# ImIntheMiddle/VATL4Pose-WACV2024

Measured on AMD Instinct MI355X. Metric: frames/sec pose-infer+uncertainty, 256x192 17-kp, higher is better.
Workload: dtype f32; 1 GPU; SimpleBaseline-R50 256x192 inference + decode + local-peak + THC-L1, 1024-frame synthetic video per GPU; frames_per_gpu=1024, batch=1024, tracks=4, parallelism=frame-sharded x1

## Files before the change

### include/vatl_hip.h

```cpp
#ifndef VATL_HIP_H
#define VATL_HIP_H

#include <stdint.h>

#ifdef __cplusplus
extern "C" {
#endif

#define VATL_VERSION 100
#define VATL_EINVAL  (-1)
#define VATL_ELAUNCH (-2)

int         vatl_version(void);
const char* vatl_last_error(void);

int vatl_flop_meter_begin(void);
int vatl_flop_meter_end(double* direct_flops, double* winograd_flops, int64_t* direct_launches, int64_t* winograd_launches);
#define VATL_ROUTE_NAMES "igemm,igemm_bnbwd,igemm_dma,persistent_1x1,streamk,rows_1x1,bottleneck_chain,stem_pool,halo_3x3," \
                         "winograd,winograd_2h,winograd_bnbwd,winograd_persist,winograd_c32,wgrad,winograd_wgrad,winograd_wgrad_2h," \
                         "winograd_wgrad_table,winograd_f4,winograd_f4_bnbwd,gemm1x1_ring"
int vatl_flop_meter_routes(int64_t* counts, int n);


int vatl_nchw_to_nhwc(const float* src, float* dst, int N, int C, int H, int W, int Cpad, void* stream);
int vatl_nhwc_to_nchw(const float* src, float* dst, int N, int C, int H, int W, void* stream);

int vatl_pack_conv_weight(const float* w_oihw, float* w_packed, int Cout, int Cin, int R, int S,
                          int CoutPad, int Spad, int CinPad, void* stream);
int vatl_pack_deconv4x4s2_weight(const float* w_iohw, float* w_packed, int Cin, int Cout, int CoutPad, void* stream);
int64_t vatl_stem_pool_weight_floats(void);
int vatl_pack_stem_pool_weight(const float* w_oihw, float* packed, void* stream);
int vatl_stem_pool_supported(int H, int W);
int vatl_stem7x7s2_pool_fwd(const float* x_nchw, const float* w_packed, const float* scale, const float* bias, float* y_nhwc,
                            int N, int H, int W, void* stream);
int64_t vatl_stem3_weight_floats(void);
int vatl_pack_stem3_weight(const float* w_oihw, float* packed, void* stream);
int vatl_stem3x3s2_fwd(const float* x_nchw, const float* w_packed, const float* scale, const float* bias, float* y_nhwc,
                       int N, int H, int W, void* stream);

int vatl_bn_fold(const float* gamma, const float* beta, const float* mean, const float* var, const float* conv_bias,
                 float eps, float* scale, float* bias, int C, void* stream);


int vatl_pack_conv1x1_dual_weight(const float* w1, const float* scale1, const float* bias1, const float* w2, const float* scale2,
                                  const float* bias2, float* out, float* bias, int Cout, int C1, int C2, int CoutPad, void* stream);
int vatl_conv1x1_dual_fwd(const float* a, const float* x, const float* w, const float* bias, float* y, int N, int Ho, int Wo,
                          int C1, int H2, int W2, int C2, int stride2, int Cout, int CoutPad, int relu, void* stream);

int64_t vatl_winograd_c32_weight_floats(void);
int vatl_pack_winograd_c32_weight(const float* w, float* u, void* stream);
int vatl_conv3x3_winograd_c32_supported(int N, int H, int W, int Cin, int Cout);
int vatl_conv3x3_winograd_c32_fwd(const float* x, const float* u, const float* scale, const float* bias, const float* residual, float* y, int N, int H, int W,
                                  int relu, void* stream);

int64_t vatl_winograd_f4_weight_floats(int Cout, int Cin);
int vatl_pack_winograd_f4_weight(const float* w, float* u, int Cout, int Cin, int data_gradient, void* stream);
int vatl_conv3x3_winograd_f4_supported(int N, int H, int W, int Cin, int Cout);
int vatl_conv3x3_winograd_f4_fwd(const float* x, const float* u, const float* scale, const float* bias, const float* residual, float* y, int N, int H, int W,
                                 int Cin, int Cout, int relu, void* stream);
int64_t vatl_winograd_f4_stats_row_blocks(int64_t N, int H, int W);
int vatl_conv3x3_winograd_f4_fwd_stats(const float* x, const float* u, float* y, double* stats, int64_t* row_blocks_used, int N, int H, int W, int Cin, int Cout,
                                       void* stream);
int vatl_conv3x3_winograd_f4_fwd_bnbwd(const float* x, const float* u, const float* residual, float* y, int N, int H, int W, int Cin, int Cout, const float* bn_z,
                                       const float* bn_mask_y, const float* bn_scale, const float* bn_bias, const float* bn_mean, const float* bn_invstd,
                                       double* stats, int64_t* row_blocks_used, void* stream);

int vatl_conv1x1_rows_supported(int K1, int K2, int N, int64_t M);
int vatl_conv1x1_rows_fwd(const float* a, const float* x2, const float* w, const float* scale, const float* bias, const float* residual, float* y,
                          int64_t M, int K1, int K2, int N, int relu, void* stream);

int vatl_bottleneck_chain_supported(int Cmid, int Cout, int Cnext, int64_t M);
int vatl_bottleneck_chain_fwd(const float* a, const float* w3, const float* scale3, const float* bias3, const float* skip, float* t,
                              const float* w1, const float* scale1, const float* bias1, float* y1, int64_t M, int Cmid, int Cout,
// ... 200 lines not shown
```

### vatl4pose-wacv2024_amd/csrc/common.h

```cpp
#pragma once
#include <hip/hip_runtime.h>
#include <atomic>
#include <cstdarg>
#include <cstdio>
#include <cstdint>

#include "vatl_hip.h"

namespace vatl {

char* err_buf();
int fail(int code, const char* fmt, ...);

void meter_add(int kind, double flops);
enum MeterRoute {
    kRouteIgemm = 0, kRouteIgemmBnBwd, kRouteIgemmDma, kRoutePersistent1x1, kRouteStreamK, kRouteRows, kRouteChain, kRouteStemPool, kRouteHalo,
    kRouteWino, kRouteWino2H, kRouteWinoBnBwd, kRouteWinoPersist, kRouteWinoC32, kRouteWgrad, kRouteWinoWgrad, kRouteWinoWgrad2H,
    kRouteWinoWgradTable, kRouteWinoF4, kRouteWinoF4BnBwd, kRouteGemm1x1Ring, kRouteCount
};
void meter_route(int route);

inline int check_launch(const char* what) {
    hipError_t e = hipGetLastError();
    if (e != hipSuccess) return fail(VATL_ELAUNCH, "%s: %s", what, hipGetErrorString(e));
    return 0;
}

inline int ensure_dynamic_lds(const void* kern, int bytes, std::atomic<unsigned>& done_mask, const char* what) {
    int d = 0;
    if (hipGetDevice(&d) != hipSuccess) return fail(VATL_ELAUNCH, "%s: no current device", what);
    const unsigned bit = 1u << (d & 31);
    if (done_mask.load(std::memory_order_acquire) & bit) return 0;
    hipError_t e = hipFuncSetAttribute(kern, hipFuncAttributeMaxDynamicSharedMemorySize, bytes);
    if (e != hipSuccess) return fail(VATL_ELAUNCH, "hipFuncSetAttribute(%s): %s", what, hipGetErrorString(e));
    done_mask.fetch_or(bit, std::memory_order_release);
    return 0;
}

static inline int cdiv(int64_t a, int64_t b) { return (int)((a + b - 1) / b); }

typedef float f32x4 __attribute__((ext_vector_type(4)));
typedef float f32x16 __attribute__((ext_vector_type(16)));

__device__ __forceinline__ void lds_barrier() {
    asm volatile("s_waitcnt lgkmcnt(0)" ::: "memory");
    __builtin_amdgcn_s_barrier();
    asm volatile("" ::: "memory");
}

__device__ __forceinline__ float wave_sum(float v) {
#pragma unroll
    for (int o = 32; o > 0; o >>= 1) v += __shfl_xor(v, o, 64);
    return v;
}
__device__ __forceinline__ double wave_sum(double v) {
#pragma unroll
    for (int o = 32; o > 0; o >>= 1) v += __shfl_xor(v, o, 64);
    return v;
}
__device__ __forceinline__ float wave_max(float v) {
#pragma unroll
    for (int o = 32; o > 0; o >>= 1) v = fmaxf(v, __shfl_xor(v, o, 64));
    return v;
}
__device__ __forceinline__ int wave_sum(int v) {
#pragma unroll
    for (int o = 32; o > 0; o >>= 1) v += __shfl_xor(v, o, 64);
    return v;
}

__device__ __forceinline__ int fast_div(int q, float inv_w) { return (int)(((float)q + 0.5f) * inv_w); }
// ... 16 lines not shown
```

### vatl4pose-wacv2024_amd/csrc/conv_igemm.hip

```cpp
#include "common.h"

#include <algorithm>
#include <atomic>
#include <cstdlib>

namespace vatl {

struct ConvParams {
    const float* x;
    const float* w;
    const float* scale;
    const float* bias;
    const float* res;
    float* y;
    int N, H, W, Cin;
    int Cout, CoutPad;
    int R, S, stride, pad_y, pad_x;
    int Ho, Wo, M;
    int OH, OW, osy, osx, ooy, oox;
    int relu, out_nchw, deconv;
    int kpr;
    int ktiles;
    int n_tiles, m_tiles;
    int order;
// ... 1052 lines not shown

    constexpr int NG = BK / 8;
    constexpr int MPG = 4 * TM * TN;
    for (int kt = 0; kt < p.ktiles; ++kt) {
        const int buf = kt & 1;
        f32x4 af[2][TM], bf[2][TN];
        frag_read(af[0], bf[0], buf, 0);
#pragma unroll
        for (int g = 0; g < NG; ++g) {
            if (g + 1 < NG) frag_read(af[(g + 1) & 1], bf[(g + 1) & 1], buf, g + 1);
            if (g == 0) issue(buf ^ 1, kt + 1);
#pragma unroll
            for (int tt = 0; tt < 4; ++tt)
#pragma unroll
                for (int i = 0; i < TM; ++i)
#pragma unroll
                    for (int j = 0; j < TN; ++j)
                        acc[i][j] = __builtin_amdgcn_mfma_f32_32x32x2f32(af[g & 1][i][tt], bf[g & 1][j][tt], acc[i][j], 0, 0, 0);
            if (g + 1 < NG) __builtin_amdgcn_sched_group_barrier(0x100, TM + TN, 0);
#pragma unroll
            for (int q2 = 0; q2 < MPG; ++q2) {
                __builtin_amdgcn_sched_group_barrier(0x008, 1, 0);
                __builtin_amdgcn_sched_group_barrier(0x016, 2, 0);
            }
            __builtin_amdgcn_sched_barrier(0);
        }
        asm volatile("s_waitcnt vmcnt(0)" ::: "memory");
        __syncthreads();
    }
    conv_epilogue<BM, BN, WM, WN>(p, acc, smem, m0, n0, ooy, oox, wm, wn, tid, lane, HoWo);
}

template <int BM, int BN, int WM, int WN>
__global__ __launch_bounds__(256, 2) void conv_igemm_dma_kernel(ConvParams p) {
    extern __shared__ __attribute__((aligned(16))) float smem[];
    conv_igemm_dma_body<BM, BN, WM, WN>(p, smem);
}

constexpr int RING_BK = 16;
constexpr int RING_NS = 4;
constexpr int RING_STAGE = 256 * RING_BK;
constexpr int RING_BYTES = RING_NS * RING_STAGE * (int)sizeof(float);

template <int N>
__device__ __forceinline__ void ring_wait_vm() {
    static_assert(N == 0 || N == 4 || N == 8 || N == 32 || N == 36, "add the count here");
    if constexpr (N == 0) asm volatile("s_waitcnt vmcnt(0)" ::: "memory");
    else if constexpr (N == 4) asm volatile("s_waitcnt vmcnt(4)" ::: "memory");
    else if constexpr (N == 8) asm volatile("s_waitcnt vmcnt(8)" ::: "memory");
    else if constexpr (N == 32) asm volatile("s_waitcnt vmcnt(32)" ::: "memory");
    else asm volatile("s_waitcnt vmcnt(36)" ::: "memory");
}

template <bool DUAL, bool RES>
__device__ __forceinline__ void gemm1x1_ring_body(const ConvParams& p, float* smem) {
    const int tid = threadIdx.x, lane = tid & 63;
    const int wave = __builtin_amdgcn_readfirstlane(tid >> 6);
    const int wm = wave >> 1, wn = wave & 1;

    const int nblk = gridDim.x, bid = blockIdx.x;
    const int xcd = bid & 7, loc = bid >> 3, q = nblk >> 3, r8 = nblk & 7;
    const int t = (xcd < r8 ? xcd * (q + 1) : r8 * (q + 1) + (xcd - r8) * q) + loc;
    const int m_tile = t / p.n_tiles, n_tile = t - m_tile * p.n_tiles;
    const int m0 = m_tile * 128, n0 = n_tile * 128;

    const __amdgpu_buffer_rsrc_t xr = __builtin_amdgcn_make_buffer_rsrc(const_cast<float*>(p.x), 0, p.x_bytes, 0x00020000);
    const __amdgpu_buffer_rsrc_t wr = __builtin_amdgcn_make_buffer_rsrc(const_cast<float*>(p.w), 0, p.w_bytes, 0x00020000);
    const __amdgpu_buffer_rsrc_t xr2 = __builtin_amdgcn_make_buffer_rsrc(const_cast<float*>(DUAL ? p.x2 : p.x), 0, DUAL ? p.x2_bytes : p.x_bytes, 0x00020000);

    const int lchk = (lane & 3) ^ ((lane >> 4) & 3);
    unsigned aoff[2], boff[2], aoff2[2];
#pragma unroll
    for (int u = 0; u < 2; ++u) {
        const int row = (4 * u + wave) * 16 + (lane >> 2);
        const int m = min(m0 + row, p.M - 1);
        aoff[u] = (unsigned)m * (unsigned)(p.Cin * 4) + (unsigned)lchk * 16u;
        aoff2[u] = 0;
        if (DUAL) {
            const int b = fdiv(m, p.d_HoWo);
            const int rem = m - b * p.Ho * p.Wo;
            const int oy = fdiv(rem, p.d_Wo);
            const int ox = rem - oy * p.Wo;
            aoff2[u] = (unsigned)((b * p.H2 + oy * p.stride2) * p.W2 + ox * p.stride2) * (unsigned)(p.C2 * 4) + (unsigned)lchk * 16u;
        }
        boff[u] = (unsigned)(n0 + row) * (unsigned)(p.K * 4) + (unsigned)lchk * 16u;
    }
    const int S = p.ktiles * 2;
    const int S1 = DUAL ? p.k1 * 2 : S;
    auto issue = [&](auto src, int buf, int s) {
        float* st = smem + buf * RING_STAGE;
#pragma unroll
        for (int u = 0; u < 2; ++u) {
            lds_void* da = (lds_void*)(st + (4 * u + wave) * 256);
            if constexpr (DUAL && decltype(src)::value == 1) __builtin_amdgcn_raw_ptr_buffer_load_lds(xr2, da, 16, aoff2[u], (unsigned)(s - S1) * 64u, 0, 0);
            else                                             __builtin_amdgcn_raw_ptr_buffer_load_lds(xr, da, 16, aoff[u], (unsigned)s * 64u, 0, 0);
        }
#pragma unroll
        for (int u = 0; u < 2; ++u)
            __builtin_amdgcn_raw_ptr_buffer_load_lds(wr, (lds_void*)(st + 128 * RING_BK + (4 * u + wave) * 256), 16, boff[u], (unsigned)s * 64u, 0, 0);
    };

    const int frow = lane & 31, h = lane >> 5;
    const int fsw = (frow >> 2) & 3;
    const float* Ard[2];
    const float* Brd[2];
#pragma unroll
    for (int g = 0; g < 2; ++g) {
        Ard[g] = smem + (wm * 64 + frow) * RING_BK + (((2 * g + h) ^ fsw) << 2);
        Brd[g] = smem + 128 * RING_BK + (wn * 64 + frow) * RING_BK + (((2 * g + h) ^ fsw) << 2);
    }

    const unsigned rowb = (unsigned)p.Cout * 4u;
    const unsigned ylane = (unsigned)(m0 + wm * 64 + 4 * h) * rowb + (unsigned)(n0 + wn * 64 + frow) * 4u;
    float sc[2], bi[2];
#pragma unroll
    for (int j = 0; j < 2; ++j) {
        const int n = n0 + wn * 64 + j * 32 + frow;
        sc[j] = p.scale ? p.scale[n] : 1.f;
        bi[j] = p.bias ? p.bias[n] : 0.f;
    }
    const __amdgpu_buffer_rsrc_t yr = __builtin_amdgcn_make_buffer_rsrc(p.y, 0, p.y_bytes, 0x00020000);
    const __amdgpu_buffer_rsrc_t rr = __builtin_amdgcn_make_buffer_rsrc(const_cast<float*>(RES ? p.res : p.y), 0, RES ? p.y_bytes : 0u, 0x00020000);
    float rs[2][2][16];
#pragma unroll
    for (int i = 0; i < 2; ++i)
#pragma unroll
        for (int j = 0; j < 2; ++j)
#pragma unroll
            for (int e = 0; e < 16; ++e) rs[i][j][e] = 0.f;
    auto res_load = [&](int i) {
#pragma unroll
        for (int j = 0; j < 2; ++j)
#pragma unroll
            for (int e = 0; e < 16; ++e)
                rs[i][j][e] = __builtin_bit_cast(float, __builtin_amdgcn_raw_buffer_load_b32(
                                  rr, ylane + (unsigned)(32 * i + (e & 3) + 8 * (e >> 2)) * rowb + (unsigned)j * 128u, 0, 0));
    };

    f32x16 acc[2][2];
#pragma unroll
    for (int i = 0; i < 2; ++i)
#pragma unroll
        for (int j = 0; j < 2; ++j)
#pragma unroll
            for (int e = 0; e < 16; ++e) acc[i][j][e] = 0.f;

    auto stage = [&](auto slot, auto kind, auto src, int s) {
        constexpr int B = decltype(slot)::value, KIND = decltype(kind)::value;
        if constexpr (KIND <= 1) ring_wait_vm<8>();
        else if constexpr (KIND == 2) ring_wait_vm<RES ? 36 : 4>();
        else ring_wait_vm<RES ? 32 : 0>();
        __builtin_amdgcn_s_barrier();
        asm volatile("" ::: "memory");
        f32x4 af[2][2], bf[2][2];
#pragma unroll
        for (int g = 0; g < 2; ++g)
#pragma unroll
            for (int i = 0; i < 2; ++i) {
                af[g][i] = *reinterpret_cast<const f32x4*>(Ard[g] + B * RING_STAGE + i * 32 * RING_BK);
                bf[g][i] = *reinterpret_cast<const f32x4*>(Brd[g] + B * RING_STAGE + i * 32 * RING_BK);
            }
        if constexpr (KIND == 0) issue(src, (B + 3) & 3, s + 3);
        if constexpr (RES && KIND == 1) res_load(0);
        if constexpr (RES && KIND == 3) res_load(1);
#pragma unroll
        for (int g = 0; g < 2; ++g)
#pragma unroll
            for (int tt = 0; tt < 4; ++tt)
#pragma unroll
                for (int i = 0; i < 2; ++i)
#pragma unroll
                    for (int j = 0; j < 2; ++j)
                        acc[i][j] = __builtin_amdgcn_mfma_f32_32x32x2f32(af[g][i][tt], bf[g][j][tt], acc[i][j], 0, 0, 0);
        __builtin_amdgcn_sched_group_barrier(0x100, 8, 0);
        if constexpr (KIND == 0) {
#pragma unroll
            for (int k = 0; k < 4; ++k) {
                __builtin_amdgcn_sched_group_barrier(0x008, 1, 0);
                __builtin_amdgcn_sched_group_barrier(0x020, 1, 0);
            }
            __builtin_amdgcn_sched_group_barrier(0x008, 28, 0);
        }
        __builtin_amdgcn_sched_barrier(0);
    };
    using C0 = std::integral_constant<int, 0>;
    using C1 = std::integral_constant<int, 1>;
    using C2 = std::integral_constant<int, 2>;
    using C3 = std::integral_constant<int, 3>;

    using X2 = std::integral_constant<int, DUAL ? 1 : 0>;
    auto group = [&](auto src, int s) {
        stage(C0{}, C0{}, src, s);
        stage(C1{}, C0{}, src, s + 1);
        stage(C2{}, C0{}, src, s + 2);
        stage(C3{}, C0{}, src, s + 3);
    };

    issue(C0{}, 0, 0);
    issue(C0{}, 1, 1);
    issue(C0{}, 2, 2);
    int s = 0;
    if constexpr (DUAL) {
        for (; s < S1 - 4; s += 4) group(C0{}, s);
        stage(C0{}, C0{}, C0{}, s);
        stage(C1{}, C0{}, X2{}, s + 1);
        stage(C2{}, C0{}, X2{}, s + 2);
        stage(C3{}, C0{}, X2{}, s + 3);
        s += 4;
    }
    for (; s < S - 4; s += 4) group(X2{}, s);
    stage(C0{}, C0{}, X2{}, s);
    stage(C1{}, C1{}, X2{}, s + 1);
    stage(C2{}, C2{}, X2{}, s + 2);
    stage(C3{}, C3{}, X2{}, s + 3);

    const float lo = p.relu ? 0.f : -INFINITY;
#pragma unroll
    for (int i = 0; i < 2; ++i)
#pragma unroll
        for (int j = 0; j < 2; ++j)
#pragma unroll
            for (int e = 0; e < 16; ++e) {
                const float v = fmaxf(acc[i][j][e] * sc[j] + bi[j] + rs[i][j][e], lo);
                __builtin_amdgcn_raw_buffer_store_b32(__builtin_bit_cast(unsigned, v), yr,
                                                      ylane + (unsigned)(32 * i + (e & 3) + 8 * (e >> 2)) * rowb + (unsigned)j * 128u, 0, 0);
            }
}

template <bool DUAL, bool RES>
__global__ __launch_bounds__(256, 2) void gemm1x1_ring_kernel(ConvParams p) {
    extern __shared__ __attribute__((aligned(16))) float smem[];
    gemm1x1_ring_body<DUAL, RES>(p, smem);
}

template <int BM, int BN, int WM, int WN>
static int launch_dma(const ConvParams& p, int phases, hipStream_t st);

static std::atomic<int> g_var{4};
static std::atomic<int> g_order{0};
static std::atomic<int> g_ablate{0};
static std::atomic<int> g_bm{0};
static std::atomic<int> g_stagger{0};
static std::atomic<int> g_splitk_policy{0};

__global__ void splitk_reduce_kernel(const float* __restrict__ part, long long slice, int splits, const float* __restrict__ scale,
                                     const float* __restrict__ bias, const float* __restrict__ res, float* __restrict__ y, long long total, int Cout,
                                     int OHW, int relu, int out_nchw) {
    for (long long i = blockIdx.x * (long long)blockDim.x + threadIdx.x; i < total; i += (long long)gridDim.x * blockDim.x) {
        const int c = (int)(i % Cout);
        float v = 0.f;
        for (int z = 0; z < splits; ++z) v += part[(long long)z * slice + i];
        v = v * (scale ? scale[c] : 1.f) + (bias ? bias[c] : 0.f);
        long long o = i;
        if (out_nchw) {
            const long long pix = i / Cout;
            const long long b = pix / OHW;
            o = (b * Cout + c) * OHW + (pix - b * OHW);
        }
        if (res) v += res[o];
        y[o] = relu ? fmaxf(v, 0.f) : v;
    }
}

constexpr int kMaxDevices = 16;
static std::atomic<float*> g_splitk_ws[kMaxDevices];
static std::atomic<long long> g_splitk_floats[kMaxDevices];
static std::atomic<int> g_splitk_any{0};

static thread_local float* tl_splitk_ws = nullptr;
static thread_local long long tl_splitk_floats = 0;

static float* splitk_workspace(long long* floats, int* policy) {
    if (tl_splitk_ws) { *floats = tl_splitk_floats; *policy = 1; return tl_splitk_ws; }
    *policy = g_splitk_policy.load(std::memory_order_relaxed);
    if (!g_splitk_any.load(std::memory_order_acquire)) return nullptr;
    int d = 0;
    if (hipGetDevice(&d) != hipSuccess || d < 0 || d >= kMaxDevices) return nullptr;
    *floats = g_splitk_floats[d].load(std::memory_order_relaxed);
    return g_splitk_ws[d].load(std::memory_order_acquire);
}

template <int BM, int BN, int WM, int WN, bool STEM, int VAR, bool DUAL = false, int NT = 256, bool BNB = false>
static int launch(const ConvParams& p, int phases, hipStream_t st) {
    auto kern = conv_igemm_kernel<BM, BN, WM, WN, STEM, VAR, DUAL, NT, BNB>;
    constexpr int smem = conv_smem_floats(BM, BN) * (int)sizeof(float);
// ... 58 lines not shown
    auto kern = conv_igemm_dma_kernel<BM, BN, WM, WN>;
    constexpr int stage_bytes = 2 * (BM + BN) * BK * (int)sizeof(float);
    constexpr int epi_bytes = BM * (BN + 4) * (int)sizeof(float);
    constexpr int smem = stage_bytes > epi_bytes ? stage_bytes : epi_bytes;
    static std::atomic<unsigned> configured{0};
    if (int rc = ensure_dynamic_lds(reinterpret_cast<const void*>(kern), smem, configured, "conv_igemm_dma")) return rc;
    ConvParams q = p;
    q.n_tiles = p.CoutPad / BN;
    q.m_tiles = cdiv(p.M, BM);
    q.order = 0; q.stagger = 0;
    dim3 grid((unsigned)(q.m_tiles * q.n_tiles), (unsigned)phases, 1);
    hipLaunchKernelGGL(kern, grid, dim3(256), smem, st, q);
    meter_add(0, 2.0 * ((double)q.m_tiles * BM) * ((double)q.n_tiles * BN) * ((double)q.ktiles * BK) * phases);
    meter_route(kRouteIgemmDma);
    return check_launch("conv_igemm_dma");
}

static std::atomic<int> g_persist_dist{2};

template <int BM, int BN, int WM, int WN, bool D2>
static int launch_persistent_impl(const ConvParams& p, hipStream_t st) {
    auto kern = gemm1x1_persistent_kernel<BM, BN, WM, WN>;
    auto kern2 = gemm1x1_persistent2_kernel<BM, BN, WM, WN>;
    constexpr int smem = conv_smem_floats(BM, BN) * (int)sizeof(float);
    static std::atomic<unsigned> configured{0};
    if (int rc = ensure_dynamic_lds(D2 ? reinterpret_cast<const void*>(kern2) : reinterpret_cast<const void*>(kern), smem, configured, "gemm1x1_persistent")) return rc;
    ConvParams q = p;
    q.n_tiles = p.CoutPad / BN;
    q.m_tiles = cdiv(p.M, BM);
    const int total = q.m_tiles * q.n_tiles;
    int grid = 512;
    if (grid > total) grid = (total + 7) / 8 * 8;
#ifdef VATL_ABLATION
    q.ablate = g_ablate.load(std::memory_order_relaxed);
    if (q.ablate & 4) q.y_bytes = 0;
    if (q.ablate & 8) q.x_bytes = 0;
    if ((q.ablate & 2) && q.ktiles > 2) { q.ktiles = 2; }
#endif
    if (D2) hipLaunchKernelGGL(kern2, dim3((unsigned)grid), dim3(256), smem, st, q);
    else    hipLaunchKernelGGL(kern, dim3((unsigned)grid), dim3(256), smem, st, q);
    meter_add(0, 2.0 * ((double)q.m_tiles * BM) * ((double)q.n_tiles * BN) * ((double)q.ktiles * BK));
    meter_route(kRoutePersistent1x1);
    return check_launch("gemm1x1_persistent");
}

template <int BM, int BN, int WM, int WN>
static int launch_persistent(const ConvParams& p, hipStream_t st) {
    const bool d2 = g_persist_dist.load(std::memory_order_relaxed) == 2 && p.ktiles >= 2 && (p.ktiles & 1) == 0;
    return d2 ? launch_persistent_impl<BM, BN, WM, WN, true>(p, st) : launch_persistent_impl<BM, BN, WM, WN, false>(p, st);
}

static std::atomic<int> g_persist{1};
static std::atomic<int> g_ring{1};

template <bool DUAL, bool RES>
static int launch_ring_impl(const ConvParams& p, hipStream_t st) {
    auto kern = gemm1x1_ring_kernel<DUAL, RES>;
    static std::atomic<unsigned> configured{0};
    if (int rc = ensure_dynamic_lds(reinterpret_cast<const void*>(kern), RING_BYTES, configured, "gemm1x1_ring")) return rc;
    ConvParams q = p;
    q.n_tiles = p.CoutPad / 128;
    q.m_tiles = cdiv(p.M, 128);
    q.splits = 1;
    hipLaunchKernelGGL(kern, dim3((unsigned)(q.m_tiles * q.n_tiles)), dim3(256), RING_BYTES, st, q);
    meter_add(0, 2.0 * ((double)q.m_tiles * 128) * ((double)q.n_tiles * 128) * ((double)q.ktiles * BK));
    meter_route(kRouteGemm1x1Ring);
    return check_launch("gemm1x1_ring");
}

static int launch_ring(const ConvParams& p, hipStream_t st) {
    if (p.x2) return launch_ring_impl<true, false>(p, st);
    return p.res ? launch_ring_impl<false, true>(p, st) : launch_ring_impl<false, false>(p, st);
}

static bool ring_wanted(const ConvParams& p, int phases, int bn, int bm, int var) {
    if (!g_ring.load(std::memory_order_relaxed) || var != 4 || phases != 1 || bn != 128 || bm != 128) return false;
    if (p.R != 1 || p.S != 1 || p.stride != 1 || p.pad_y || p.pad_x || p.out_nchw || p.deconv || p.stats || p.bz) return false;
    if (p.osy != 1 || p.osx != 1 || p.OH != p.Ho || p.OW != p.Wo || p.H != p.Ho || p.W != p.Wo) return false;
    if (p.Cout != p.CoutPad || (p.ktiles & 1) || p.ktiles < (p.x2 ? 12 : 16)) return false;
    if (p.x2 && (p.res || p.k1 < 2 || (p.k1 & 1) || p.ktiles - p.k1 < 2)) return false;
    if ((long long)(p.M + 128) * p.Cout >= (1LL << 30)) return false;
    long long ws_floats = 0;
    int sk_policy = 0;
    return splitk_workspace(&ws_floats, &sk_policy) == nullptr;
}

constexpr int kStreamKGrid = 768;
constexpr long long kStreamKBytes = 4096 + (long long)kStreamKGrid * 64 * 128 * 4;
static thread_local char* tl_streamk_ws = nullptr;
static thread_local unsigned tl_streamk_epoch = 0;
static std::atomic<int> g_streamk{1};

template <bool BNB>
static int launch_streamk(const ConvParams& p, hipStream_t st) {
    auto kern = conv_streamk_kernel<64, 128, 32, 64, BNB>;
    constexpr int smem = conv_smem_floats(64, 128) * (int)sizeof(float);
    static std::atomic<unsigned> configured{0};
    if (int rc = ensure_dynamic_lds(reinterpret_cast<const void*>(kern), smem, configured, "conv_streamk")) return rc;
    ConvParams q = p;
    q.n_tiles = p.CoutPad / 128;
    q.m_tiles = cdiv(p.M, 64);
    q.splits = 1;
    StreamKArgs sk{};
    sk.flags = reinterpret_cast<unsigned*>(tl_streamk_ws);
    sk.slabs = reinterpret_cast<float*>(tl_streamk_ws + 4096);
    sk.epoch = ++tl_streamk_epoch;
    if (sk.epoch == 0) sk.epoch = ++tl_streamk_epoch;
    sk.tiles = q.m_tiles * q.n_tiles;
    hipLaunchKernelGGL(kern, dim3(kStreamKGrid), dim3(256), smem, st, q, sk);
    meter_add(0, 2.0 * ((double)q.m_tiles * 64) * ((double)q.n_tiles * 128) * ((double)q.ktiles * BK));
    meter_route(kRouteStreamK);
    return check_launch("conv_streamk");
}

static bool streamk_wanted(const ConvParams& p, int phases, int bn, int bm, bool stem) {
    if (!tl_streamk_ws || !g_streamk.load(std::memory_order_relaxed) || stem || phases != 1 || bn != 128 || bm != 64 || p.x2 || p.out_nchw || p.deconv ||
        (p.Cout & 3) || p.ktiles < 8)
        return false;
    const long long tiles = (long long)cdiv(p.M, 64) * (p.CoutPad / 128);
    const long long rounds = (tiles + kStreamKGrid - 1) / kStreamKGrid;
    if (tiles * 100 >= rounds * kStreamKGrid * 85) return false;
    return tiles * p.ktiles >= 6LL * kStreamKGrid && tiles >= 64;
}

static int tile_n_for(int Cout) { return Cout <= 32 ? 32 : (Cout <= 64 ? 64 : 128); }

static int tile_m_for(const ConvParams& p, int phases, int bn, bool stem) {
    if (stem || bn < 64) return 128;
    const int forced = g_bm.load(std::memory_order_relaxed);
    if (forced == 64 || forced == 128) return forced;
    const long long blocks128 = (long long)cdiv(p.M, 128) * (p.CoutPad / bn) * phases;
    if (bn == 64) return blocks128 >= 1536 ? 128 : 64;
    return blocks128 < 768 ? 64 : 128;
// ... 70 lines not shown
                     int Cin, int Cout, int CoutPad, int R, int S, int stride, int pad, int relu, hipStream_t st);
int conv3x3_halo_enable(int on);
int wino_set_ablate(int bits);
int wino_set_group_kb(int v);
int wino_set_halves(int v);
int wino_set_persist(int v);
int wino_wgrad_set_halves(int v);
int wino_wgrad_set_table(int v);
int wino_set_persist_pf(int v);
int wino_wgrad_set_blocks(int v);

}

using namespace vatl;

namespace vatl {
__attribute__((visibility("hidden"))) int tune_wgrad_blocks(int blocks);
__attribute__((visibility("hidden"))) int crop_tune_px(int px);
}

extern "C" int vatl_tune_set(int knob, int value) {
    switch (knob) {
    case 0:  if (value == 0 || value == 2 || value == 4 || value == 5) { g_var.store(value, std::memory_order_relaxed); return 0; } break;
    case 1:  if (value == 0 || value == 1) { g_order.store(value, std::memory_order_relaxed); return 0; } break;
    case 5:  if (value == 0 || value == 64 || value == 128) { g_bm.store(value, std::memory_order_relaxed); return 0; } break;
    case 7:  if (value >= 0 && value <= 64) { g_persist.store(value, std::memory_order_relaxed); return 0; } break;
    case 8:  if (value == 0 || value == 1) return conv3x3_halo_enable(value); break;
    case 10: if (value == 1 || value == 2) { g_persist_dist.store(value, std::memory_order_relaxed); return 0; } break;
    case 18: if (value >= 0 && value <= (1 << 20)) return wino_set_group_kb(value); break;
    case 21: if (value >= 1 && value <= 3) return wino_set_halves(value); break;
    case 22: if (value >= 0 && value <= 4096) return wino_set_persist(value); break;
    case 24: if (value >= 0 && value <= 3) return wino_set_persist_pf(value); break;
    case 25: if (value == 0 || value == 1) return wino_wgrad_set_table(value); break;
    default: break;
    }
#ifdef VATL_ABLATION
    const bool wrong = (knob == 0 && value >= 10) || ((knob == 4 || knob == 6 || knob == 17) && value != 0);
    if (wrong) {
        const char* ok = getenv("VATL_ALLOW_ABLATION");
        if (!ok || ok[0] != '1') return fail(VATL_EINVAL, "tune_set: knob %d value %d is a profiling ablation (wrong results); set VATL_ALLOW_ABLATION=1", knob, value);
    }
    if (knob == 0 && value >= 10 && value <= 13) { g_var.store(value, std::memory_order_relaxed); return 0; }
    if (knob == 2 && value >= 0 && value <= 200) { g_stagger.store(value, std::memory_order_relaxed); return 0; }
    if (knob == 3 && tune_wgrad_blocks(value) == 0) return 0;
    if (knob == 4 && value >= 0 && value <= 3) return tune_wgrad_blocks(-value - 1);
    if (knob == 6 && value >= 0 && value <= 15) { g_ablate.store(value, std::memory_order_relaxed); return 0; }
    if (knob == 9 && (value == 0 || value == 1)) { g_splitk_policy.store(value, std::memory_order_relaxed); return 0; }
    if (knob == 12 && (value == 0 || value == 1)) { g_streamk.store(value, std::memory_order_relaxed); return 0; }
    if (knob == 16 && crop_tune_px(value) == 0) return 0;
    if (knob == 17 && value >= 0 && value <= 63) return wino_set_ablate(value);
    if (knob == 19 && value >= 1 && value <= (1 << 20)) return wino_wgrad_set_blocks(value);
    if (knob == 23 && value >= 1 && value <= 2) return wino_wgrad_set_halves(value);
    if (knob == 27 && (value == 0 || value == 1)) { g_ring.store(value, std::memory_order_relaxed); return 0; }
    return fail(VATL_EINVAL, "tune_set: unknown knob %d / value %d", knob, value);
#else
    return fail(VATL_EINVAL, "tune_set: knob %d / value %d is not a product knob (include/vatl_hip.h lists them: 0, 1, 5, 7, 8, 10, 18, 21, 22, 24, 25 — all bit-identical); "
                "knobs that change the summation order, performance experiments and profiling ablations exist only in the variant built with "
                "`build.py --ablation` (-DVATL_ABLATION)", knob, value);
#endif
}

extern "C" int vatl_set_splitk_workspace_thread(float* workspace, int64_t floats) {
    if (workspace && floats <= 0) return fail(VATL_EINVAL, "set_splitk_workspace_thread: empty workspace");
    tl_splitk_ws = workspace;
    tl_splitk_floats = workspace ? (long long)floats : 0;
    return 0;
}

extern "C" int64_t vatl_streamk_workspace_bytes(void) { return kStreamKBytes; }

extern "C" int vatl_set_streamk_workspace_thread(void* workspace, int64_t bytes) {
    if (workspace && bytes < kStreamKBytes) return fail(VATL_EINVAL, "set_streamk_workspace_thread: %lld bytes, need %lld", (long long)bytes, kStreamKBytes);
    tl_streamk_ws = static_cast<char*>(workspace);
    return 0;
}

extern "C" int vatl_set_splitk_workspace(float* workspace, int64_t floats) {
    if (workspace && floats <= 0) return fail(VATL_EINVAL, "set_splitk_workspace: empty workspace");
    int d = 0;
    if (hipGetDevice(&d) != hipSuccess || d < 0 || d >= kMaxDevices) return fail(VATL_EINVAL, "set_splitk_workspace: no current device (or index >= %d)", kMaxDevices);
    g_splitk_floats[d].store(workspace ? (long long)floats : 0, std::memory_order_relaxed);
    g_splitk_ws[d].store(workspace, std::memory_order_release);
    int any = 0;
    for (int i = 0; i < kMaxDevices; ++i) any |= g_splitk_ws[i].load(std::memory_order_relaxed) != nullptr;
    g_splitk_any.store(any, std::memory_order_release);
    return 0;
}

extern "C" int vatl_conv_cout_pad(int Cout) {
    const int bn = tile_n_for(Cout);
    return (Cout + bn - 1) / bn * bn;
}

static int conv2d_fwd_impl(const float* x, const float* w, const float* scale, const float* bias, const float* residual,
                           float* y, int N, int H, int W, int Cin, int Cout, int CoutPad, int R, int S, int stride, int pad,
                           int relu, int out_nchw, double* stats, int64_t* row_blocks, void* stream) {
    if (!x || !w || !y || N <= 0) return fail(VATL_EINVAL, "conv2d_fwd: null pointer or empty batch");
    if (stats && ((Cout & 3) || out_nchw)) return fail(VATL_EINVAL, "conv2d_fwd_stats: Cout %d must be a multiple of 4 (NHWC output)", Cout);
    const bool stem = (Cin == 4);
    if (!stem && Cin % 32 != 0) return fail(VATL_EINVAL, "conv2d_fwd: Cin %d must be a multiple of 32 (or 4 for the stem)", Cin);
    if (!stats && !out_nchw) {
        const int rc = conv3x3_halo_try(x, w, scale, bias, residual, y, N, H, W, Cin, Cout, CoutPad, R, S, stride, pad, relu, (hipStream_t)stream);
        if (rc <= 0) return rc;
    }
    if (stem && S > 8) return fail(VATL_EINVAL, "conv2d_fwd: stem filter width %d > 8", S);
    ConvParams p{};
// ... 134 lines not shown
```

### vatl4pose-wacv2024_amd/vatl_hip/__init__.py

```python
from __future__ import annotations

import ctypes as C
import os

import torch

_HERE = os.path.dirname(os.path.abspath(__file__))
LIB_PATH = os.environ.get("VATL_HIP_LIB") or os.path.join(_HERE, "libvatl_hip.so")

_p = C.c_void_p
_i = C.c_int
_f = C.c_float
_d = C.c_double
_i64 = C.c_int64

SIGNATURES = {
    "vatl_version": (_i, []),
    "vatl_last_error": (C.c_char_p, []),
    "vatl_flop_meter_begin": (_i, []),
    "vatl_flop_meter_end": (_i, [_p, _p, _p, _p]),
    "vatl_flop_meter_routes": (_i, [_p, _i]),
    "vatl_nchw_to_nhwc": (_i, [_p, _p, _i, _i, _i, _i, _i, _p]),
    "vatl_nhwc_to_nchw": (_i, [_p, _p, _i, _i, _i, _i, _p]),
    "vatl_pack_conv_weight": (_i, [_p, _p, _i, _i, _i, _i, _i, _i, _i, _p]),
# ... 145 lines not shown
        raise VatlError(f"{what} failed ({rc}): {lib().vatl_last_error().decode()}")


def upload(host, device, dtype=None, owned: bool = False):
    t = torch.as_tensor(host)
    device = torch.device(device)
    if t.is_cuda:
        return t.to(device=device, dtype=dtype if dtype is not None else t.dtype)
    if dtype is not None and t.dtype != dtype:
        t = t.to(dtype)
    if device.type != "cuda" or t.numel() == 0:
        return t.to(device)
    if owned and t.is_pinned() and t.is_contiguous():
        return t.to(device, non_blocking=True)
    stage = torch.empty(t.shape, dtype=t.dtype, pin_memory=True)
    stage.copy_(t)
    return stage.to(device, non_blocking=True)


def _ptr(t, dtype=torch.float32):
    if t is None:
        return None
    if not t.is_cuda:
        raise VatlError("vatl_hip needs device (HIP) tensors; there is no CPU path")
    if t.dtype != dtype:
        raise VatlError(f"expected {dtype}, got {t.dtype}")
    if not t.is_contiguous():
        raise VatlError("tensor must be contiguous")
    return t.data_ptr()


def _stream():
    return torch.cuda.current_stream().cuda_stream



def nchw_to_nhwc(x: torch.Tensor, cpad: int | None = None) -> torch.Tensor:
    n, c, h, w = x.shape
    cpad = cpad or c
    y = torch.empty((n, h, w, cpad), device=x.device, dtype=torch.float32)
    _check(lib().vatl_nchw_to_nhwc(_ptr(x), _ptr(y), n, c, h, w, cpad, _stream()), "vatl_nchw_to_nhwc")
    return y


def nhwc_to_nchw(x: torch.Tensor) -> torch.Tensor:
    n, h, w, c = x.shape
    y = torch.empty((n, c, h, w), device=x.device, dtype=torch.float32)
    _check(lib().vatl_nhwc_to_nchw(_ptr(x), _ptr(y), n, c, h, w, _stream()), "vatl_nhwc_to_nchw")
    return y


ROUTE_NAMES = ("igemm", "igemm_bnbwd", "igemm_dma", "persistent_1x1", "streamk", "rows_1x1", "bottleneck_chain", "stem_pool", "halo_3x3", "winograd",
               "winograd_2h", "winograd_bnbwd", "winograd_persist", "winograd_c32", "wgrad", "winograd_wgrad", "winograd_wgrad_2h", "winograd_wgrad_table", "winograd_f4", "winograd_f4_bnbwd",
               "gemm1x1_ring")


class flop_meter:

    def __enter__(self):
        _check(lib().vatl_flop_meter_begin(), "flop_meter_begin")
        self.direct = self.winograd = self.total = 0.0
        self.direct_launches = self.winograd_launches = 0
        return self

    @staticmethod
    def launches_now() -> int:
        counts = (C.c_int64 * len(ROUTE_NAMES))()
        _check(min(0, lib().vatl_flop_meter_routes(counts, len(ROUTE_NAMES))), "flop_meter_routes")
        return int(sum(counts))

    def __exit__(self, *exc):
        counts = (C.c_int64 * len(ROUTE_NAMES))()
        _check(min(0, lib().vatl_flop_meter_routes(counts, len(ROUTE_NAMES))), "flop_meter_routes")
        self.routes = {n: int(c) for n, c in zip(ROUTE_NAMES, counts)}
        d, w, nd, nw = C.c_double(0), C.c_double(0), C.c_int64(0), C.c_int64(0)
        _check(lib().vatl_flop_meter_end(C.byref(d), C.byref(w), C.byref(nd), C.byref(nw)), "flop_meter_end")
        self.direct, self.winograd, self.total = d.value, w.value, d.value + w.value
        self.direct_launches, self.winograd_launches = nd.value, nw.value
        return False


def tune_set(knob: int, value: int):
    _check(lib().vatl_tune_set(knob, value), "vatl_tune_set")


_splitk_buf = {}


def enable_splitk(megabytes: int = 64, device=None):
    dev = torch.device(device) if device is not None else torch.device("cuda", torch.cuda.current_device())
    idx = dev.index if dev.index is not None else torch.cuda.current_device()
    with torch.cuda.device(idx):
        if megabytes <= 0:
            _check(lib().vatl_set_splitk_workspace(None, 0), "vatl_set_splitk_workspace")
            _splitk_buf.pop(idx, None)
            return
        buf = torch.empty(megabytes * (1 << 18), device=torch.device("cuda", idx), dtype=torch.float32)
        _check(lib().vatl_set_splitk_workspace(_ptr(buf), buf.numel()), "vatl_set_splitk_workspace")
        _splitk_buf[idx] = buf


_splitk_scratch = {}
_splitk_scratch_lock = __import__("threading").Lock()
SPLITK_SCRATCH_MB = 256


class splitk_scope:
# ... 1140 lines not shown
```

Before: 16480 frames/s.

## Extend LDS ring GEMM kernel to stride-2 3x3 convolutions via per-tap offsets

Generalizes the 1x1 ring-buffered GEMM kernel (buffer_load_lds with a 4-stage LDS ring) to 3x3 stride-2 pad-1 convolutions. The K loop walks the nine filter taps, recomputes per-row input offsets at each tap boundary, and points out-of-bounds taps at the buffer end so the hardware returns zero. This is meant to give the ResNet downsampling 3x3 convs the same asynchronous global-to-LDS pipelining the 1x1 layers already use. The tap transitions add extra bookkeeping and require Cin to be a multiple of 64, and the eligibility rules for the 1x1 path are reorganized.

```diff
diff --git a/include/vatl_hip.h b/include/vatl_hip.h
--- a/include/vatl_hip.h
+++ b/include/vatl_hip.h
@@ -18,7 +18,7 @@
 int vatl_flop_meter_end(double* direct_flops, double* winograd_flops, int64_t* direct_launches, int64_t* winograd_launches);
 #define VATL_ROUTE_NAMES "igemm,igemm_bnbwd,igemm_dma,persistent_1x1,streamk,rows_1x1,bottleneck_chain,stem_pool,halo_3x3," \
                          "winograd,winograd_2h,winograd_bnbwd,winograd_persist,winograd_c32,wgrad,winograd_wgrad,winograd_wgrad_2h," \
-                         "winograd_wgrad_table,winograd_f4,winograd_f4_bnbwd,gemm1x1_ring"
+                         "winograd_wgrad_table,winograd_f4,winograd_f4_bnbwd,gemm1x1_ring,conv3x3_ring"
 int vatl_flop_meter_routes(int64_t* counts, int n);
 
 
diff --git a/vatl4pose-wacv2024_amd/csrc/common.h b/vatl4pose-wacv2024_amd/csrc/common.h
--- a/vatl4pose-wacv2024_amd/csrc/common.h
+++ b/vatl4pose-wacv2024_amd/csrc/common.h
@@ -16,7 +16,7 @@
 enum MeterRoute {
     kRouteIgemm = 0, kRouteIgemmBnBwd, kRouteIgemmDma, kRoutePersistent1x1, kRouteStreamK, kRouteRows, kRouteChain, kRouteStemPool, kRouteHalo,
     kRouteWino, kRouteWino2H, kRouteWinoBnBwd, kRouteWinoPersist, kRouteWinoC32, kRouteWgrad, kRouteWinoWgrad, kRouteWinoWgrad2H,
-    kRouteWinoWgradTable, kRouteWinoF4, kRouteWinoF4BnBwd, kRouteGemm1x1Ring, kRouteCount
+    kRouteWinoWgradTable, kRouteWinoF4, kRouteWinoF4BnBwd, kRouteGemm1x1Ring, kRouteConv3x3Ring, kRouteCount
 };
 void meter_route(int route);
 
diff --git a/vatl4pose-wacv2024_amd/csrc/conv_igemm.hip b/vatl4pose-wacv2024_amd/csrc/conv_igemm.hip
--- a/vatl4pose-wacv2024_amd/csrc/conv_igemm.hip
+++ b/vatl4pose-wacv2024_amd/csrc/conv_igemm.hip
@@ -1128,8 +1128,9 @@
     else asm volatile("s_waitcnt vmcnt(36)" ::: "memory");
 }
 
-template <bool DUAL, bool RES>
+template <bool DUAL, bool RES, bool TAPS = false>
 __device__ __forceinline__ void gemm1x1_ring_body(const ConvParams& p, float* smem) {
+    static_assert(!(DUAL && TAPS), "one second offset set");
     const int tid = threadIdx.x, lane = tid & 63;
     const int wave = __builtin_amdgcn_readfirstlane(tid >> 6);
     const int wm = wave >> 1, wn = wave & 1;
@@ -1146,12 +1147,24 @@
 
     const int lchk = (lane & 3) ^ ((lane >> 4) & 3);
     unsigned aoff[2], boff[2], aoff2[2];
+    int iy0[2], ix0[2];
+    unsigned pix[2];
 #pragma unroll
     for (int u = 0; u < 2; ++u) {
         const int row = (4 * u + wave) * 16 + (lane >> 2);
         const int m = min(m0 + row, p.M - 1);
         aoff[u] = (unsigned)m * (unsigned)(p.Cin * 4) + (unsigned)lchk * 16u;
         aoff2[u] = 0;
+        iy0[u] = 0; ix0[u] = 0; pix[u] = 0;
+        if (TAPS) {
+            const int b = fdiv(m, p.d_HoWo);
+            const int rem = m - b * p.Ho * p.Wo;
+            const int oy = fdiv(rem, p.d_Wo);
+            const int ox = rem - oy * p.Wo;
+            iy0[u] = oy * p.stride - p.pad_y;
+            ix0[u] = ox * p.stride - p.pad_x;
+            pix[u] = (unsigned)((b * p.H + iy0[u]) * p.W + ix0[u]) * (unsigned)(p.Cin * 4) + (unsigned)lchk * 16u;
+        }
         if (DUAL) {
             const int b = fdiv(m, p.d_HoWo);
             const int rem = m - b * p.Ho * p.Wo;
@@ -1161,15 +1174,24 @@
         }
         boff[u] = (unsigned)(n0 + row) * (unsigned)(p.K * 4) + (unsigned)lchk * 16u;
     }
+    auto set_tap = [&](unsigned (&dst)[2], int tr, int ts) {
+#pragma unroll
+        for (int u = 0; u < 2; ++u) {
+            const bool in = (unsigned)(iy0[u] + tr) < (unsigned)p.H && (unsigned)(ix0[u] + ts) < (unsigned)p.W;
+            dst[u] = in ? pix[u] + (unsigned)((tr * p.W + ts) * p.Cin) * 4u : p.x_bytes;
+        }
+    };
+    if (TAPS) set_tap(aoff, 0, 0);
     const int S = p.ktiles * 2;
     const int S1 = DUAL ? p.k1 * 2 : S;
+    int sb0 = 0, sb1 = DUAL ? S1 : 0;
     auto issue = [&](auto src, int buf, int s) {
         float* st = smem + buf * RING_STAGE;
 #pragma unroll
         for (int u = 0; u < 2; ++u) {
             lds_void* da = (lds_void*)(st + (4 * u + wave) * 256);
-            if constexpr (DUAL && decltype(src)::value == 1) __builtin_amdgcn_raw_ptr_buffer_load_lds(xr2, da, 16, aoff2[u], (unsigned)(s - S1) * 64u, 0, 0);
-            else                                             __builtin_amdgcn_raw_ptr_buffer_load_lds(xr, da, 16, aoff[u], (unsigned)s * 64u, 0, 0);
+            if constexpr ((DUAL || TAPS) && decltype(src)::value == 1) __builtin_amdgcn_raw_ptr_buffer_load_lds(xr2, da, 16, aoff2[u], (unsigned)(s - sb1) * 64u, 0, 0);
+            else                                                       __builtin_amdgcn_raw_ptr_buffer_load_lds(xr, da, 16, aoff[u], (unsigned)(s - sb0) * 64u, 0, 0);
         }
 #pragma unroll
         for (int u = 0; u < 2; ++u)
@@ -1271,6 +1293,12 @@
         stage(C2{}, C0{}, src, s + 2);
         stage(C3{}, C0{}, src, s + 3);
     };
+    auto cross = [&](int s) {
+        stage(C0{}, C0{}, C0{}, s);
+        stage(C1{}, C0{}, C1{}, s + 1);
+        stage(C2{}, C0{}, C1{}, s + 2);
+        stage(C3{}, C0{}, C1{}, s + 3);
+    };
 
     issue(C0{}, 0, 0);
     issue(C0{}, 1, 1);
@@ -1278,11 +1306,22 @@
     int s = 0;
     if constexpr (DUAL) {
         for (; s < S1 - 4; s += 4) group(C0{}, s);
-        stage(C0{}, C0{}, C0{}, s);
-        stage(C1{}, C0{}, X2{}, s + 1);
-        stage(C2{}, C0{}, X2{}, s + 2);
-        stage(C3{}, C0{}, X2{}, s + 3);
+        cross(s);
         s += 4;
+    }
+    if constexpr (TAPS) {
+        const int spt = p.Cin / RING_BK;
+        int tr = 0, ts = 0;
+        for (int tap = 1; tap < p.R * p.S; ++tap) {
+            if (++ts == p.S) { ts = 0; ++tr; }
+            set_tap(aoff2, tr, ts);
+            sb1 = sb0 + spt;
+            for (; s < sb1 - 4; s += 4) group(C0{}, s);
+            cross(s);
+            s += 4;
+            aoff[0] = aoff2[0]; aoff[1] = aoff2[1];
+            sb0 = sb1;
+        }
     }
     for (; s < S - 4; s += 4) group(X2{}, s);
     stage(C0{}, C0{}, X2{}, s);
@@ -1307,6 +1346,11 @@
 __global__ __launch_bounds__(256, 2) void gemm1x1_ring_kernel(ConvParams p) {
     extern __shared__ __attribute__((aligned(16))) float smem[];
     gemm1x1_ring_body<DUAL, RES>(p, smem);
+}
+
+__global__ __launch_bounds__(256, 2) void conv3x3_ring_kernel(ConvParams p) {
+    extern __shared__ __attribute__((aligned(16))) float smem[];
+    gemm1x1_ring_body<false, false, true>(p, smem);
 }
 
 template <int BM, int BN, int WM, int WN>
@@ -1471,33 +1515,43 @@
 
 static std::atomic<int> g_persist{1};
 static std::atomic<int> g_ring{1};
-
-template <bool DUAL, bool RES>
+static std::atomic<int> g_ring3{1};
+
+template <bool DUAL, bool RES, bool TAPS = false>
 static int launch_ring_impl(const ConvParams& p, hipStream_t st) {
-    auto kern = gemm1x1_ring_kernel<DUAL, RES>;
+    auto kern = TAPS ? conv3x3_ring_kernel : gemm1x1_ring_kernel<DUAL, RES>;
+    const char* what = TAPS ? "conv3x3_ring" : "gemm1x1_ring";
     static std::atomic<unsigned> configured{0};
-    if (int rc = ensure_dynamic_lds(reinterpret_cast<const void*>(kern), RING_BYTES, configured, "gemm1x1_ring")) return rc;
+    if (int rc = ensure_dynamic_lds(reinterpret_cast<const void*>(kern), RING_BYTES, configured, what)) return rc;
     ConvParams q = p;
     q.n_tiles = p.CoutPad / 128;
     q.m_tiles = cdiv(p.M, 128);
     q.splits = 1;
     hipLaunchKernelGGL(kern, dim3((unsigned)(q.m_tiles * q.n_tiles)), dim3(256), RING_BYTES, st, q);
     meter_add(0, 2.0 * ((double)q.m_tiles * 128) * ((double)q.n_tiles * 128) * ((double)q.ktiles * BK));
-    meter_route(kRouteGemm1x1Ring);
-    return check_launch("gemm1x1_ring");
+    meter_route(TAPS ? kRouteConv3x3Ring : kRouteGemm1x1Ring);
+    return check_launch(what);
 }
 
 static int launch_ring(const ConvParams& p, hipStream_t st) {
+    if (p.R != 1) return launch_ring_impl<false, false, true>(p, st);
     if (p.x2) return launch_ring_impl<true, false>(p, st);
     return p.res ? launch_ring_impl<false, true>(p, st) : launch_ring_impl<false, false>(p, st);
 }
 
 static bool ring_wanted(const ConvParams& p, int phases, int bn, int bm, int var) {
-    if (!g_ring.load(std::memory_order_relaxed) || var != 4 || phases != 1 || bn != 128 || bm != 128) return false;
-    if (p.R != 1 || p.S != 1 || p.stride != 1 || p.pad_y || p.pad_x || p.out_nchw || p.deconv || p.stats || p.bz) return false;
-    if (p.osy != 1 || p.osx != 1 || p.OH != p.Ho || p.OW != p.Wo || p.H != p.Ho || p.W != p.Wo) return false;
-    if (p.Cout != p.CoutPad || (p.ktiles & 1) || p.ktiles < (p.x2 ? 12 : 16)) return false;
-    if (p.x2 && (p.res || p.k1 < 2 || (p.k1 & 1) || p.ktiles - p.k1 < 2)) return false;
+    if (var != 4 || phases != 1 || bn != 128 || bm != 128) return false;
+    if (p.out_nchw || p.deconv || p.stats || p.bz) return false;
+    if (p.osy != 1 || p.osx != 1 || p.OH != p.Ho || p.OW != p.Wo || p.Cout != p.CoutPad) return false;
+    if (p.R == 3) {
+        if (!g_ring3.load(std::memory_order_relaxed) || p.S != 3 || p.stride != 2 || p.pad_y != 1 || p.pad_x != 1) return false;
+        if (p.x2 || p.res || p.Cin % 64 || (unsigned long long)p.x_bytes + (unsigned)p.Cin * 4u >= (1ULL << 32)) return false;
+    } else {
+        if (!g_ring.load(std::memory_order_relaxed)) return false;
+        if (p.R != 1 || p.S != 1 || p.stride != 1 || p.pad_y || p.pad_x || p.H != p.Ho || p.W != p.Wo) return false;
+        if ((p.ktiles & 1) || p.ktiles < (p.x2 ? 12 : 16)) return false;
+        if (p.x2 && (p.res || p.k1 < 2 || (p.k1 & 1) || p.ktiles - p.k1 < 2)) return false;
+    }
     if ((long long)(p.M + 128) * p.Cout >= (1LL << 30)) return false;
     long long ws_floats = 0;
     int sk_policy = 0;
@@ -1674,6 +1728,7 @@
     if (knob == 19 && value >= 1 && value <= (1 << 20)) return wino_wgrad_set_blocks(value);
     if (knob == 23 && value >= 1 && value <= 2) return wino_wgrad_set_halves(value);
     if (knob == 27 && (value == 0 || value == 1)) { g_ring.store(value, std::memory_order_relaxed); return 0; }
+    if (knob == 28 && (value == 0 || value == 1)) { g_ring3.store(value, std::memory_order_relaxed); return 0; }
     return fail(VATL_EINVAL, "tune_set: unknown knob %d / value %d", knob, value);
 #else
     return fail(VATL_EINVAL, "tune_set: knob %d / value %d is not a product knob (include/vatl_hip.h lists them: 0, 1, 5, 7, 8, 10, 18, 21, 22, 24, 25 — all bit-identical); "
diff --git a/vatl4pose-wacv2024_amd/vatl_hip/__init__.py b/vatl4pose-wacv2024_amd/vatl_hip/__init__.py
--- a/vatl4pose-wacv2024_amd/vatl_hip/__init__.py
+++ b/vatl4pose-wacv2024_amd/vatl_hip/__init__.py
@@ -221,7 +221,7 @@
 
 ROUTE_NAMES = ("igemm", "igemm_bnbwd", "igemm_dma", "persistent_1x1", "streamk", "rows_1x1", "bottleneck_chain", "stem_pool", "halo_3x3", "winograd",
                "winograd_2h", "winograd_bnbwd", "winograd_persist", "winograd_c32", "wgrad", "winograd_wgrad", "winograd_wgrad_2h", "winograd_wgrad_table", "winograd_f4", "winograd_f4_bnbwd",
-               "gemm1x1_ring")
+               "gemm1x1_ring", "conv3x3_ring")
 
 
 class flop_meter:
```

Result: no change. 16580 frames/s (median of 6 runs) (+0.6%).
